# yerfor/Real3DPortrait

Hardware: AMD Instinct MI355X
Metric: rendered frames/sec @ 512x512, 48 depth samples (higher is better)
Workload: dtype f32 operands as fp16 hi + lo, fp32 accumulate (SR precision 'f16mx' = the library default, superresolution.DEFAULT_SR_PRECISION; the fp32-class f16x3 is `alt_f16x3`): in block0.conv1, block1.conv0 and block1.conv1 hi*hi runs on the f16 MFMA and the two cross products on the block-scaled 8-bit MFMA

## Files before the change

real3dportrait_amd/csrc/r3d_sr_f16x3.hip:

```cpp
#include <stdlib.h>

#include "r3d_sr_common.h"
#include "r3d_stamps.h"

namespace r3d {

typedef _Float16 h8 __attribute__((ext_vector_type(8)));
typedef _Float16 h4 __attribute__((ext_vector_type(4)));
static constexpr int F_TILE_H = 16, F_TILE_W = 16;
static constexpr int F_PATCH_H = F_TILE_H + 2, F_PATCH_W = F_TILE_W + 2, F_PATCH_PIX = F_PATCH_H * F_PATCH_W;

__device__ __forceinline__ void split1(float v, _Float16& hi, _Float16& lo)
{
    v = as_rounded(v);
    const float c = fminf(fmaxf(v, -65504.f), 65504.f);
    hi = (_Float16)c;
    lo = (_Float16)(v - (float)hi);
}

__device__ __forceinline__ void split1_folded(float v, _Float16& hi, _Float16& lo)
{
    v = as_rounded(v);
    hi = (_Float16)v;
    lo = (_Float16)(v - (float)hi);
}

__device__ __host__ __forceinline__ int mx_rec_chan(int dword) { return 8 * (dword & 1) + 4 * (dword >> 1); }
static constexpr float kMxWl = 256.0f , kMxWh = 0.125f ;
static constexpr int kMxFmtB = 1;
static constexpr int kMxScaleA = 127, kMxScaleB = 119;
static constexpr float kMxXh = 1.0f, kMxXl = 2048.0f ;

__device__ __forceinline__ unsigned pack4_fp8(float a, float b, float c, float d)
{
    int v = 0;
    v = __builtin_amdgcn_cvt_pk_fp8_f32(a, b, v, false);
    v = __builtin_amdgcn_cvt_pk_fp8_f32(c, d, v, true);
    return (unsigned)v;
}
__device__ __forceinline__ unsigned pack4_x8(float a, float b, float c, float d)
{
    int v = 0;
    v = __builtin_amdgcn_cvt_pk_bf8_f32(a, b, v, false);
    v = __builtin_amdgcn_cvt_pk_bf8_f32(c, d, v, true);
    return (unsigned)v;
}

__global__ void weight_row_stats_kernel(const float* __restrict__ w, int row_len, int CoutReal, int Cout, float* __restrict__ tail)
{
    const int co = blockIdx.x;
    const ConvTail T = conv_tail_layout(Cout);
    float mx = 0.f, l1 = 0.f;
    if (co < CoutReal)
// ... 794 lines not shown
    auto issue_w = [&](int st, u32x4& r) { r = *reinterpret_cast<const u32x4*>(WP + (size_t)(st < nst ? st : nst - 1) * 4 * a.Cout); };
    uint4* const Abuf = lds + 2 * BL_PATCH;
    const int aoff = h * 256 + 64 * wm + li;
    const int prow = li >> 4, row0 = wn * 2 * NT;
    int boff[NT];
#pragma unroll
    for (int nt = 0; nt < NT; ++nt) boff[nt] = h * 256 + (row0 + nt * 2 + prow) * 16 + (li & 15);

#pragma unroll
    for (int d = 0; d < BL_DEPTH; ++d) { issue(d, raw[d]); issue_w(d, wraw[d]); }
    stage_patch(0, raw[0], lds);
    *reinterpret_cast<u32x4*>(Abuf + threadIdx.x) = wraw[0];
    issue(BL_DEPTH, raw[0]); issue_w(BL_DEPTH, wraw[0]);
    asm volatile("s_waitcnt lgkmcnt(0)" ::: "memory");
    __builtin_amdgcn_s_barrier();
    asm volatile("" ::: "memory");
    for (int s0 = 0; s0 < nst; s0 += BL_DEPTH) {
#pragma unroll
        for (int d = 0; d < BL_DEPTH; ++d) {
            const int s = s0 + d;
            {
                const uint4* P = lds + (d & 1) * BL_PATCH;
                const uint4* A = Abuf + (d & 1) * 512 + aoff;
                h8 ah[2], al[2];
#pragma unroll
                for (int mt = 0; mt < 2; ++mt) { const uint4 q0 = A[32 * mt], q1 = A[128 + 32 * mt]; ah[mt] = *reinterpret_cast<const h8*>(&q0); al[mt] = *reinterpret_cast<const h8*>(&q1); }
                h8 bh[NT], bl[NT];
#pragma unroll
                for (int nt = 0; nt < NT; ++nt) { const uint4 r0 = P[boff[nt]], r1 = P[512 + boff[nt]]; bh[nt] = *reinterpret_cast<const h8*>(&r0); bl[nt] = *reinterpret_cast<const h8*>(&r1); }
#pragma unroll
                for (int nt = 0; nt < NT; ++nt)
#pragma unroll
                    for (int mt = 0; mt < 2; ++mt) {
                        acc[mt][nt] = __builtin_amdgcn_mfma_f32_32x32x16_f16(al[mt], bh[nt], acc[mt][nt], 0, 0, 0);
                        acc[mt][nt] = __builtin_amdgcn_mfma_f32_32x32x16_f16(ah[mt], bl[nt], acc[mt][nt], 0, 0, 0);
                        acc[mt][nt] = __builtin_amdgcn_mfma_f32_32x32x16_f16(ah[mt], bh[nt], acc[mt][nt], 0, 0, 0);
                    }
                stage_patch(s + 1, raw[(d + 1) % BL_DEPTH], lds + ((d + 1) & 1) * BL_PATCH);
                *reinterpret_cast<u32x4*>(Abuf + ((d + 1) & 1) * 512 + threadIdx.x) = wraw[(d + 1) % BL_DEPTH];
                issue(s + 1 + BL_DEPTH, raw[(d + 1) % BL_DEPTH]); issue_w(s + 1 + BL_DEPTH, wraw[(d + 1) % BL_DEPTH]);
                asm volatile("s_waitcnt lgkmcnt(0)" ::: "memory");
                __builtin_amdgcn_s_barrier();
                asm volatile("" ::: "memory");
            }
        }
    }
    conv_epilogue<WN, NT>(a, ph, n, acc, i0, j0, m0, reinterpret_cast<float*>(lds));
}

static constexpr int U_TILE = 14;
static constexpr int U_WSTAGE = 9 * 2 * 2 * 32;
static constexpr int U_PW = 17, U_PPLANE = 320;
static constexpr int U_PATCH = 4 * U_PPLANE;
static constexpr int U_STAGE = U_PATCH + U_WSTAGE;
static constexpr int U_LDS_UINT4 = 2 * U_STAGE + 2;
static constexpr int U_ZERO = 2 * U_STAGE;


struct UpArgs {
    const uint4* x; size_t x_stride_n;
    const uint4* wp;
    const float* out_scale; const float* bias; const float* next_scale; size_t vec_stride_n;
    uint4* y; size_t y_stride_n;
    int Cin, Cout, H, W, tiles_x, ntiles, tiles_per_xcd;
    float clamp;
    unsigned long long* clk;
};

__global__ void sr_prepack_up_kernel(const float* __restrict__ w, int Cin, int Cout, const float* __restrict__ winv, uint4* __restrict__ out)
{
    const size_t e = (size_t)blockIdx.x * blockDim.x + threadIdx.x;
    const size_t total = (size_t)9 * (Cin / 8) * Cout * 2;
    if (e >= total) return;
    const int co = e & 31, hl = (e >> 5) & 1, hc = (e >> 6) & 1;
    const int t = (int)((e >> 7) % 9);
    const size_t r = (e >> 7) / 9;
    const int nst = Cin / 16;
    const int st = (int)(r % nst), cg = (int)(r / nst);
    const int cout = cg * 32 + co;
    h8 v8;
#pragma unroll
    for (int j = 0; j < 8; ++j) {
        const int ci = st * 16 + hc * 8 + j;
        _Float16 a, b; split1(w[((size_t)cout * Cin + ci) * 9 + t] * (1.0f / winv[cout]), a, b);
        v8[j] = hl ? b : a;
    }
    out[e] = *reinterpret_cast<uint4*>(&v8);
}

__global__ void sr_prepack_up_mx_kernel(const float* __restrict__ w, int Cin, int Cout, const float* __restrict__ winv, uint4* __restrict__ out)
{
    const size_t e = (size_t)blockIdx.x * blockDim.x + threadIdx.x;
    const size_t total = (size_t)9 * (Cin / 8) * Cout * 2;
    if (e >= total) return;
    const int co = e & 31, hl = (e >> 5) & 1, hc = (e >> 6) & 1;
    const int t = (int)((e >> 7) % 9);
    const size_t r = (e >> 7) / 9;
    const int nst = Cin / 16;
    const int st = (int)(r % nst), cg = (int)(r / nst);
    const int cout = cg * 32 + co;
    const float ws = 1.0f / winv[cout];
    if (!hl) {
        h8 v8;
#pragma unroll
        for (int j = 0; j < 8; ++j) { _Float16 a, b; split1(w[((size_t)cout * Cin + st * 16 + hc * 8 + j) * 9 + t] * ws, a, b); v8[j] = a; }
        out[e] = *reinterpret_cast<uint4*>(&v8);
        return;
    }
    uint4 rec;
    unsigned* pr = reinterpret_cast<unsigned*>(&rec);
#pragma unroll
    for (int q = 0; q < 4; ++q) {
        float f[4];
#pragma unroll
        for (int j = 0; j < 4; ++j) {
            const float v = w[((size_t)cout * Cin + st * 16 + mx_rec_chan(q) + j) * 9 + t] * ws;
            _Float16 a, b; split1(v, a, b);
            f[j] = hc ? (float)a * kMxWh : (v - (float)a) * kMxWl;
        }
        pr[q] = pack4_fp8(f[0], f[1], f[2], f[3]);
    }
    out[e] = rec;
}

template <bool CLAMP, bool MX = false, bool MXIN = false, int NW = 4>
__global__ __launch_bounds__(64 * NW, NW == 8 ? 4 : 2) void upconv_fir_f16x3_kernel(UpArgs a)
{
    constexpr int NTL = 8 / NW;
    constexpr int NTHR = 64 * NW;
    R3D_STAMP_DECL;
    __shared__ uint4 lds[U_LDS_UINT4];
    const int G = a.Cout >> 5;
    const int xcd = blockIdx.x & 7, slot = blockIdx.x >> 3;
    const int tl = slot / G, cg = slot - tl * G;
    const int tile = xcd * a.tiles_per_xcd + tl;
    if (tile >= a.ntiles) return;
    const int n = blockIdx.y;
    if (blockIdx.x == (gridDim.x >> 1) && n == 0 && threadIdx.x == 0) clk_begin(kernarg_clk<UpArgs>());
    const int ty = tile / a.tiles_x, tx = tile - ty * a.tiles_x;
    const int i0 = ty * U_TILE, j0 = tx * U_TILE;
    const int tid = threadIdx.x, lane = tid & 63, wave = tid >> 6;
    const int li = lane & 31, h = lane >> 5;
    const int nst = a.Cin >> 4;
    const int chunk_stride = a.H * a.W;
    const size_t plane = (size_t)(a.Cin >> 3) * chunk_stride;
    const uint4* X = a.x + (size_t)n * a.x_stride_n;

    f32x16 acc[4][NTL];
#pragma unroll
    for (int p = 0; p < 4; ++p)
#pragma unroll
        for (int nt = 0; nt < NTL; ++nt)
#pragma unroll
            for (int r = 0; r < 16; ++r) acc[p][nt][r] = 0.f;

    const int prow = li >> 4, pcol = ((li & 15) - prow) & 15;
    const int row0 = wave * 2 * NTL;
    int boff[NTL];
#pragma unroll
    for (int nt = 0; nt < NTL; ++nt) boff[nt] = (row0 + nt * 2 + prow + 1) * U_PW + (pcol + 1) + h * U_PPLANE;
    const int aoff = U_PATCH + h * 64 + li;
    int b8c[NTL], b8r[NTL];
#pragma unroll
    for (int nt = 0; nt < NTL; ++nt) {
        const int pix = (row0 + nt * 2 + prow + 1) * U_PW + (pcol + 1) + 2 * U_PPLANE;
        b8c[nt] = pix - h; b8r[nt] = pix - h * U_PW;
    }
    const int a8d2 = U_PATCH + 32 + li + h * 256, a8d6 = U_PATCH + 32 + li + h * 768;
    const int a8c = U_PATCH + 32 + li + 4 * 128;
    if (MXIN && tid < 2) lds[U_ZERO + tid] = make_uint4(0, 0, 0, 0);

    const int wave_u = __builtin_amdgcn_readfirstlane(wave);
    constexpr int PK = (20 + NW - 1) / NW;
    constexpr int WKF = 18 / NW, WKR = 18 - WKF * NW;
    unsigned pf_off[PK];
    unsigned pf_valid = 0;
#pragma unroll
    for (int k = 0; k < PK; ++k) {
        const int sg = NW * k + wave_u, pc = sg / 5, idx = (sg - pc * 5) * 64 + lane;
        const int py = idx / U_PW, px = idx - py * U_PW;
        const int iy = i0 - 2 + py, ix = j0 - 2 + px;
        unsigned off = 0;
        if (sg < 20 && idx < U_PW * U_PW && iy >= 0 && iy < a.H && ix >= 0 && ix < a.W) {
            off = (unsigned)((pc >> 1) * plane) + (unsigned)((pc & 1) * chunk_stride + iy * a.W + ix);
            pf_valid |= 1u << k;
        }
        pf_off[k] = off;
    }
    const uint4* WP = a.wp + (size_t)cg * nst * U_WSTAGE;
    auto dma_stage = [&](int st, uint4* buf) {
        const uint4* src = WP + (size_t)st * U_WSTAGE + tid;
#pragma unroll
        for (int k = 0; k <= WKF; ++k)
            if (k < WKF || wave_u < WKR) dma64(src + NTHR * k, buf + U_PATCH + NTHR * k + 64 * wave_u);
        const uint4* Xs = X + (size_t)(2 * st) * chunk_stride;
#pragma unroll
        for (int k = 0; k < PK; ++k) {
            if (NW * k + wave_u < 20) {
                const uint4* g = (pf_valid & (1u << k)) ? Xs + pf_off[k] : g_zero16;
                dma64(g, buf + 64 * (NW * k + wave_u));
            }
        }
    };
    dma_stage(0, lds);
    R3D_STAMP(0);
    i8v pa68, pa17, pb68[NTL], pb17[NTL];
    for (int st = 0; st < nst; ++st) {
#ifdef R3D_STAMPS
        asm volatile("s_waitcnt lgkmcnt(0)" ::: "memory"); R3D_STAMP(1);
#endif
        asm volatile("s_waitcnt vmcnt(0) lgkmcnt(0)" ::: "memory");
        R3D_STAMP(4);
        __builtin_amdgcn_s_barrier();
        R3D_STAMP(5);
        asm volatile("" ::: "memory");
        const uint4* cur = lds + (st & 1) * U_STAGE;
        if (st + 1 < nst) dma_stage(st + 1, lds + ((st + 1) & 1) * U_STAGE);
        if constexpr (MXIN) {
            auto ld8 = [&](const uint4* p0, const uint4* p1) {
                const uint4 q0 = *p0, q1 = *p1;
                return (i8v){(int)q0.x, (int)q0.y, (int)q0.z, (int)q0.w, (int)q1.x, (int)q1.y, (int)q1.z, (int)q1.w};
            };
            auto ldh = [&](const uint4* p0) { uint4 q = *p0; return *reinterpret_cast<h8*>(&q); };
            const uint4* curA = cur + aoff;
            const int cb = (st & 1) * U_STAGE;
            h8 B1[2][NTL], A1[6];
#pragma unroll
            for (int nt = 0; nt < NTL; ++nt) { B1[0][nt] = ldh(cur + boff[nt]); B1[1][nt] = ldh(cur + boff[nt] - 1); }
            {
                constexpr int T1[6] = {0, 1, 3, 4, 2, 5};
#pragma unroll
                for (int k = 0; k < 6; ++k) A1[k] = ldh(curA + T1[k] * 128);
            }
            __builtin_amdgcn_sched_barrier(0);
            if (st > 0) {
#pragma unroll
                for (int nt = 0; nt < NTL; ++nt) {
                    acc[0][nt] = __builtin_amdgcn_mfma_scale_f32_32x32x64_f8f6f4(pa68, pb68[nt], acc[0][nt], 0, kMxFmtB, 0, kMxScaleA, 0, kMxScaleB);
                    acc[1][nt] = __builtin_amdgcn_mfma_scale_f32_32x32x64_f8f6f4(pa17, pb17[nt], acc[1][nt], 0, kMxFmtB, 0, kMxScaleA, 0, kMxScaleB);
                }
            }
            __builtin_amdgcn_sched_barrier(0);
            h8 B2[2][NTL], A2[3];
#pragma unroll
            for (int nt = 0; nt < NTL; ++nt) { B2[0][nt] = ldh(cur + boff[nt] - U_PW); B2[1][nt] = ldh(cur + boff[nt] - U_PW - 1); }
#pragma unroll
            for (int k = 0; k < 3; ++k) A2[k] = ldh(curA + (6 + k) * 128);
            __builtin_amdgcn_sched_barrier(0);
#pragma unroll
            for (int k = 0; k < 4; ++k)
#pragma unroll
                for (int nt = 0; nt < NTL; ++nt) acc[k][nt] = __builtin_amdgcn_mfma_f32_32x32x16_f16(A1[k], B1[0][nt], acc[k][nt], 0, 0, 0);
#pragma unroll
            for (int k = 0; k < 2; ++k)
#pragma unroll
                for (int nt = 0; nt < NTL; ++nt) acc[2 * k][nt] = __builtin_amdgcn_mfma_f32_32x32x16_f16(A1[4 + k], B1[1][nt], acc[2 * k][nt], 0, 0, 0);
            __builtin_amdgcn_sched_barrier(0);
            const i8v a02 = ld8(lds + cb + a8d2 + 0 * 128, lds + cb + a8d2 + 0 * 128 + 64);
            const i8v a35 = ld8(lds + cb + a8d2 + 3 * 128, lds + cb + a8d2 + 3 * 128 + 64);
            const i8v a4 = ld8(lds + (h ? U_ZERO : cb + a8c), lds + (h ? U_ZERO + 1 : cb + a8c + 64));
            i8v b3[NTL];
#pragma unroll
            for (int nt = 0; nt < NTL; ++nt) b3[nt] = ld8(cur + b8c[nt], cur + b8c[nt] + U_PPLANE);
            __builtin_amdgcn_sched_barrier(0);
#pragma unroll
            for (int k = 0; k < 2; ++k)
#pragma unroll
                for (int nt = 0; nt < NTL; ++nt) acc[k][nt] = __builtin_amdgcn_mfma_f32_32x32x16_f16(A2[k], B2[0][nt], acc[k][nt], 0, 0, 0);
#pragma unroll
            for (int nt = 0; nt < NTL; ++nt) acc[0][nt] = __builtin_amdgcn_mfma_f32_32x32x16_f16(A2[2], B2[1][nt], acc[0][nt], 0, 0, 0);
            __builtin_amdgcn_sched_barrier(0);
            pa68 = ld8(lds + cb + a8d2 + 6 * 128, lds + cb + a8d2 + 6 * 128 + 64);
            pa17 = ld8(lds + cb + a8d6 + 1 * 128, lds + cb + a8d6 + 1 * 128 + 64);
#pragma unroll
            for (int nt = 0; nt < NTL; ++nt) {
                pb68[nt] = ld8(cur + b8c[nt] - U_PW, cur + b8c[nt] - U_PW + U_PPLANE);
                pb17[nt] = ld8(cur + b8r[nt], cur + b8r[nt] + U_PPLANE);
            }
            __builtin_amdgcn_sched_barrier(0);
#pragma unroll
            for (int nt = 0; nt < NTL; ++nt) {
                acc[0][nt] = __builtin_amdgcn_mfma_scale_f32_32x32x64_f8f6f4(a02, b3[nt], acc[0][nt], 0, kMxFmtB, 0, kMxScaleA, 0, kMxScaleB);
                acc[2][nt] = __builtin_amdgcn_mfma_scale_f32_32x32x64_f8f6f4(a35, b3[nt], acc[2][nt], 0, kMxFmtB, 0, kMxScaleA, 0, kMxScaleB);
                acc[3][nt] = __builtin_amdgcn_mfma_scale_f32_32x32x64_f8f6f4(a4, b3[nt], acc[3][nt], 0, kMxFmtB, 0, kMxScaleA, 0, kMxScaleB);
            }
            __builtin_amdgcn_sched_barrier(0);
            continue;
        }
#pragma unroll
        for (int win = 0; win < 4; ++win) {
            const int sy = win >> 1, sx = win & 1;
            const int toff = -(sy * U_PW + sx);
            h8 bh[NTL], bl[NTL];
#pragma unroll
            for (int nt = 0; nt < NTL; ++nt) {
                uint4 r0 = cur[boff[nt] + toff];
                uint4 r1 = cur[boff[nt] + toff + 2 * U_PPLANE];
                bh[nt] = *reinterpret_cast<h8*>(&r0); bl[nt] = *reinterpret_cast<h8*>(&r1);
            }
#pragma unroll
            for (int ky = 2 * sy; ky <= (sy ? 2 : 1); ++ky)
#pragma unroll
                for (int kx = 2 * sx; kx <= (sx ? 2 : 1); ++kx) {
                    const int t = ky * 3 + kx, p = (ky & 1) * 2 + (kx & 1);
                    uint4 q0 = cur[t * 128 + aoff], q1 = cur[t * 128 + aoff + 32];
                    const h8 ah = *reinterpret_cast<h8*>(&q0), al = *reinterpret_cast<h8*>(&q1);
#pragma unroll
                    for (int nt = 0; nt < NTL; ++nt) {
                        acc[p][nt] = __builtin_amdgcn_mfma_f32_32x32x16_f16(al, bh[nt], acc[p][nt], 0, 0, 0);
                        acc[p][nt] = __builtin_amdgcn_mfma_f32_32x32x16_f16(ah, bl[nt], acc[p][nt], 0, 0, 0);
                        acc[p][nt] = __builtin_amdgcn_mfma_f32_32x32x16_f16(ah, bh[nt], acc[p][nt], 0, 0, 0);
                    }
                }
        }
    }
    if constexpr (MXIN) {
#pragma unroll
        for (int nt = 0; nt < NTL; ++nt) {
            acc[0][nt] = __builtin_amdgcn_mfma_scale_f32_32x32x64_f8f6f4(pa68, pb68[nt], acc[0][nt], 0, kMxFmtB, 0, kMxScaleA, 0, kMxScaleB);
            acc[1][nt] = __builtin_amdgcn_mfma_scale_f32_32x32x64_f8f6f4(pa17, pb17[nt], acc[1][nt], 0, kMxFmtB, 0, kMxScaleA, 0, kMxScaleB);
        }
    }

    R3D_STAMP(1);
    typedef float f2 __attribute__((ext_vector_type(2)));
    typedef _Float16 hh2 __attribute__((ext_vector_type(2)));
    float4* hls0 = reinterpret_cast<float4*>(lds);
    const int co0 = cg * 32;
    const float* D = a.out_scale + (size_t)n * a.vec_stride_n + co0;
    const float* Bv = a.bias + (size_t)n * a.vec_stride_n + co0;
    const float* NS = a.next_scale + (size_t)n * a.vec_stride_n + co0;
    const int OH = 2 * a.H, OW = 2 * a.W;
    const size_t oplane = (size_t)(a.Cout >> 3) * OH * OW;
    float4 dv4[4], bv4[4], nv4[4];
#pragma unroll
    for (int g = 0; g < 4; ++g) {
        dv4[g] = *reinterpret_cast<const float4*>(D + 8 * g + 4 * (tid & 1));
        bv4[g] = *reinterpret_cast<const float4*>(Bv + 8 * g + 4 * (tid & 1));
        nv4[g] = *reinterpret_cast<const float4*>(NS + 8 * g + 4 * (tid & 1));
    }
#pragma unroll
    for (int g = 0; g < 4; ++g)
        asm volatile("" :: "v"(dv4[g].x), "v"(dv4[g].w), "v"(bv4[g].x), "v"(bv4[g].w), "v"(nv4[g].x), "v"(nv4[g].w));
    __syncthreads();
    unsigned mxk_h[1024 / NTHR][2], mxk_l[1024 / NTHR][2];
#pragma unroll
    for (int k = 0; k < 1024 / NTHR; ++k) { mxk_h[k][0] = mxk_h[k][1] = 0u; mxk_l[k][0] = mxk_l[k][1] = 0u; }
#pragma unroll
    for (int g = 0; g < 4; ++g) {
        float4* hls = hls0 + (g & 1) * 2048;
#pragma unroll
        for (int pa = 0; pa < 2; ++pa)
#pragma unroll
            for (int nt = 0; nt < NTL; ++nt) {
                float hx[2][4];
#pragma unroll
                for (int r = 0; r < 4; ++r) {
                    const float t0 = acc[2 * pa][nt][4 * g + r], t1 = acc[2 * pa + 1][nt][4 * g + r];
                    const float ts = t0 + t1;
                    const float tsp1 = __builtin_bit_cast(float, __builtin_amdgcn_mov_dpp(__builtin_bit_cast(int, ts), 0x12F, 0xF, 0xF, true));
                    const float t0p1 = __builtin_bit_cast(float, __builtin_amdgcn_mov_dpp(__builtin_bit_cast(int, t0), 0x12F, 0xF, 0xF, true));
                    const float t1p1 = __builtin_bit_cast(float, __builtin_amdgcn_mov_dpp(__builtin_bit_cast(int, t1), 0x12F, 0xF, 0xF, true));
                    const float t0p2 = __builtin_bit_cast(float, __builtin_amdgcn_mov_dpp(__builtin_bit_cast(int, t0), 0x12E, 0xF, 0xF, true));
                    const float t1p2 = __builtin_bit_cast(float, __builtin_amdgcn_mov_dpp(__builtin_bit_cast(int, t1), 0x12E, 0xF, 0xF, true));
                    hx[0][r] = __builtin_fmaf(tsp1, 3.0f, t1 + t0p2);
                    hx[1][r] = __builtin_fmaf(t1p1 + t0p2, 3.0f, t0p1 + t1p2);
                }
                const int gy = row0 + nt * 2 + prow;
#pragma unroll
                for (int dx = 0; dx < 2; ++dx)
                    hls[((pa * 2 + h) * 16 + gy) * 32 + ((2 * pcol + dx + 8 * h) & 31)] = make_float4(hx[dx][0], hx[dx][1], hx[dx][2], hx[dx][3]);
            }
        __syncthreads();
        {
            const float4 b4 = bv4[g], n4 = nv4[g], d4 = dv4[g];
            const f2 ba = f2{b4.x, b4.y}, bb = f2{b4.z, b4.w};
            const f2 da = f2{d4.x, d4.y} * 0.0625f, db = f2{d4.z, d4.w} * 0.0625f;
            const float m = 1.4142135623730951f;
            const f2 ma = f2{n4.x, n4.y} * m, mb = f2{n4.z, n4.w} * m;
            uint4* d = a.y + (size_t)n * a.y_stride_n + (size_t)((co0 >> 3) + g) * OH * OW;
#pragma unroll
            for (int k = 0; k < 1024 / NTHR; ++k) {
                const int q = tid + NTHR * k;
                const int half = q & 1, oc = (q >> 1) & 31, rp = q >> 6;
                const bool live = rp < U_TILE && oc < 2 * U_TILE;
                f2 ha[5], hb[5];
#pragma unroll
                for (int rr = 0; rr < 5; ++rr) {
                    const int gyy = min(rp, U_TILE - 1) + ((rr + 1) >> 1);
                    const float4 t4 = hls[((((rr + 1) & 1) * 2 + half) * 16 + gyy) * 32 + ((oc + 8 * half) & 31)];
                    ha[rr] = f2{t4.x, t4.y}; hb[rr] = f2{t4.z, t4.w};
                }
#pragma unroll
                for (int dy = 0; dy < 2; ++dy) {
                    f2 va = ((ha[dy] + ha[dy + 3]) + (ha[dy + 1] + ha[dy + 2]) * 3.0f) * da + ba;
                    f2 vb = ((hb[dy] + hb[dy + 3]) + (hb[dy + 1] + hb[dy + 2]) * 3.0f) * db + bb;
                    va = __builtin_elementwise_max(va, va * 0.2f);
                    vb = __builtin_elementwise_max(vb, vb * 0.2f);
                    if constexpr (CLAMP) {
                        const f2 lim = f2{a.clamp, a.clamp} * 0.7071067811865476f;
                        va = __builtin_elementwise_min(__builtin_elementwise_max(va, -lim), lim);
                        vb = __builtin_elementwise_min(__builtin_elementwise_max(vb, -lim), lim);
                    }
                    va = va * ma;
                    vb = vb * mb;
                    asm("" : "+v"(va), "+v"(vb));
                    const hh2 hia = __builtin_convertvector(va, hh2), hib = __builtin_convertvector(vb, hh2);
                    const hh2 loa = __builtin_convertvector(va - __builtin_convertvector(hia, f2), hh2);
                    const hh2 lob = __builtin_convertvector(vb - __builtin_convertvector(hib, f2), hh2);
                    const uint2 hw = make_uint2(*reinterpret_cast<const unsigned*>(&hia), *reinterpret_cast<const unsigned*>(&hib));
                    const int oy = 2 * (i0 + rp) + dy, ox = 2 * j0 + oc;
                    if constexpr (MX) {
                        const f2 fha = __builtin_convertvector(hia, f2), fhb = __builtin_convertvector(hib, f2);
                        const f2 fla = va - fha, flb = vb - fhb;
                        const unsigned xh8 = pack4_x8(fha.x * kMxXh, fha.y * kMxXh, fhb.x * kMxXh, fhb.y * kMxXh);
                        const unsigned xl8 = pack4_x8(fla.x * kMxXl, fla.y * kMxXl, flb.x * kMxXl, flb.y * kMxXl);
                        if (!(g & 1)) { mxk_h[k][dy] = xh8; mxk_l[k][dy] = xl8; }
                        if (live && oy < OH && ox < OW) {
                            const size_t pix = (size_t)oy * OW + ox;
                            reinterpret_cast<uint2*>(d + pix)[half] = hw;
                            if (g & 1) {
                                uint4* rec = a.y + (size_t)n * a.y_stride_n + oplane + (size_t)((co0 >> 3) + (g & ~1)) * OH * OW + pix;
                                reinterpret_cast<uint2*>(rec)[half] = make_uint2(mxk_h[k][dy], xh8);
                                reinterpret_cast<uint2*>(rec + (size_t)OH * OW)[half] = make_uint2(mxk_l[k][dy], xl8);
                            }
                        }
                    } else {
                        const uint2 lw = make_uint2(*reinterpret_cast<const unsigned*>(&loa), *reinterpret_cast<const unsigned*>(&lob));
                        if (live && oy < OH && ox < OW) {
                            uint2* d2 = reinterpret_cast<uint2*>(d + (size_t)oy * OW + ox) + half;
                            d2[0] = hw;
                            d2[2 * oplane] = lw;
                        }
                    }
                }
            }
        }
    }
    R3D_STAMP(2);
    if (blockIdx.x == (gridDim.x >> 1) && blockIdx.y == 0 && threadIdx.x == 0) clk_end(kernarg_clk<UpArgs>());
#ifdef R3D_STAMPS
    asm volatile("s_waitcnt vmcnt(0)" ::: "memory");
    R3D_STAMP(3);
    R3D_STAMP_FLUSH(6, 1);
#endif
}
R3D_STAMP_READER(r3d_debug_stamps_sr)

__global__ void rgb_finalize_kernel(const float* __restrict__ img_prev, const float* __restrict__ partial, size_t part_stride_n,
                                    int nparts, const float* __restrict__ brgb, size_t vec_stride_n,
                                    float* __restrict__ img_out, uint8_t* __restrict__ img_u8, int H, int W, float clamp, int up)
{
    const int n = blockIdx.y;
    const int p = blockIdx.x * blockDim.x + threadIdx.x;
    if (p >= H * W) return;
    const int y = p / W, xx = p - y * W;
    const int Hh = H >> 1, Wh = W >> 1;
    const int ky = y >> 1, kx = xx >> 1;
    int r0, r1, c0, c1; float wy0, wy1, wx0, wx1;
    if (y & 1) { r0 = ky; r1 = ky + 1; wy0 = 0.75f; wy1 = 0.25f; } else { r0 = ky - 1; r1 = ky; wy0 = 0.25f; wy1 = 0.75f; }
    if (xx & 1) { c0 = kx; c1 = kx + 1; wx0 = 0.75f; wx1 = 0.25f; } else { c0 = kx - 1; c1 = kx; wx0 = 0.25f; wx1 = 0.75f; }
    const bool vr0 = r0 >= 0 && r0 < Hh, vr1 = r1 >= 0 && r1 < Hh, vc0 = c0 >= 0 && c0 < Wh, vc1 = c1 >= 0 && c1 < Wh;
    float rgb[3];
#pragma unroll
    for (int c = 0; c < 3; ++c) {
        float t = brgb[(size_t)n * vec_stride_n + c];
        for (int m = 0; m < nparts; ++m) t += partial[(size_t)n * part_stride_n + ((size_t)m * 3 + c) * H * W + p];
        if (clamp >= 0.f) t = fminf(fmaxf(t, -clamp), clamp);
        float upv;
        if (up) {
            const float* I = img_prev + ((size_t)n * 3 + c) * Hh * Wh;
            upv = 0.f;
            if (vr0 && vc0) upv += I[(size_t)r0 * Wh + c0] * (wy0 * wx0);
            if (vr0 && vc1) upv += I[(size_t)r0 * Wh + c1] * (wy0 * wx1);
            if (vr1 && vc0) upv += I[(size_t)r1 * Wh + c0] * (wy1 * wx0);
            if (vr1 && vc1) upv += I[(size_t)r1 * Wh + c1] * (wy1 * wx1);
        } else {
            upv = img_prev[((size_t)n * 3 + c) * H * W + p];
        }
        rgb[c] = upv + t;
        if (img_out) img_out[((size_t)n * 3 + c) * H * W + p] = rgb[c];
    }
    if (img_u8) {
        uint8_t* d = img_u8 + ((size_t)n * H * W + p) * 3;
#pragma unroll
        for (int c = 0; c < 3; ++c) d[c] = frame_u8(rgb[c]);
    }
}

__global__ void cb8_to_nchw2_kernel(const float* __restrict__ src, float* __restrict__ dst, int C, int HW)
{
    const int n = blockIdx.z, cb = blockIdx.y;
    const int p = blockIdx.x * blockDim.x + threadIdx.x;
// ... 153 lines not shown
    const size_t mu = (size_t)9 * (Cin / 8) * Cout * 2;
    hipLaunchKernelGGL(sr_prepack_up_kernel, dim3((unsigned)((mu + 255) / 256)), dim3(256), 0, st, c0_w, Cin, Cout, tail0 + T.winv,
                       reinterpret_cast<uint4*>(out + P.c0_up));
    if (mx) {
        hipLaunchKernelGGL(sr_prepack_up_mx_kernel, dim3((unsigned)((mu + 255) / 256)), dim3(256), 0, st, c0_w, Cin, Cout, tail0 + T.winv,
                           reinterpret_cast<uint4*>(out + P.c0_up_mx));
        if ((Cin & 15) == 0)
            hipLaunchKernelGGL(sr_prepack_mx_kernel, dim3((unsigned)((m0 / 2 + 255) / 256)), dim3(256), 0, st, c0_w, Cin, Cout, 9, Cin, Cout,
                               tail0 + T.winv, reinterpret_cast<uint4*>(out + P.c0_mx));
    }
    {
        const size_t mw = (size_t)(Cout >> 7) * (Cout >> 4) * 8 * 3 * 2 * 32;
        hipLaunchKernelGGL(sr_prepack_wino_kernel, dim3((unsigned)((mw + 255) / 256)), dim3(256), 0, st, c1_w, Cout, Cout, Cout, Cout, tail1 + T.winv,
                           reinterpret_cast<uint4*>(out + P.c1_wino), mx ? 1 : 0);
    }
    return check_launch("sr_block_prepack");
}

static void launch_conv2(Conv2Args& a, int tiles, int N, hipStream_t st, bool mx = false, bool wino = false)
{
    a.clk = prof_clock_slot(R3D_PROF_CONV);
    dim3 grid(tiles, a.Cout / BLOCK_M, N);
    a.order = (tiles & 7) == 0 ? 2 : 0;
    if (wino) {
        if (mx) hipLaunchKernelGGL(conv_wino_f16x3_kernel<true>, grid, dim3(512), 0, st, a);
        else hipLaunchKernelGGL(conv_wino_f16x3_kernel<false>, grid, dim3(512), 0, st, a);
        return;
    }
    if (a.ph[0].ntaps == 9 && (size_t)tiles * grid.y * grid.z <= 256) {
        const int t8 = ((a.ph[0].outW + F_TILE_W - 1) / F_TILE_W) * ((a.ph[0].outH + 7) / 8);
        a.order = (t8 & 7) == 0 ? 2 : 0;
        if (mx) hipLaunchKernelGGL(conv_mfma_f16x3_rows8_kernel<true>, dim3(t8, grid.y, grid.z), dim3(512), 0, st, a);
        else hipLaunchKernelGGL(conv_mfma_f16x3_rows8_kernel<false>, dim3(t8, grid.y, grid.z), dim3(512), 0, st, a);
        return;
    }
    if (a.ph[0].ntaps == 1) hipLaunchKernelGGL((conv1x1_mfma_f16x3_kernel<4, 2, 4>), grid, dim3(512), 0, st, a);
    else if (mx) hipLaunchKernelGGL((conv_mfma_f16x3_kernel<4, 2, 4, true>), grid, dim3(512), 0, st, a);
    else hipLaunchKernelGGL((conv_mfma_f16x3_kernel<4, 2, 4>), grid, dim3(512), 0, st, a);
}

static int tiles_of(int H, int W) { return ((W + F_TILE_W - 1) / F_TILE_W) * ((H + F_TILE_H - 1) / F_TILE_H); }

static void conv_set_output(Conv2Args& a, void* y, int y_format, int Cout, int H, int W, const float* next_scale, size_t next_scale_stride)
{
    if (y_format == R3D_FMT_CB8) { a.y_f32 = reinterpret_cast<float*>(y); a.y_f32_stride_n = (size_t)Cout * H * W; }
    else if (y_format == R3D_FMT_NCHW) { a.y_nchw = reinterpret_cast<float*>(y); a.y_nchw_stride_n = (size_t)Cout * H * W; }
    else if (y_format == R3D_FMT_SPLIT || y_format == R3D_FMT_SPLIT_MX) {
        a.y_split = reinterpret_cast<uint4*>(y); a.y_split_stride_n = (size_t)Cout / 8 * H * W * 2;
        a.next_scale = next_scale; a.next_scale_stride_n = next_scale_stride;
        a.y_split_mx = y_format == R3D_FMT_SPLIT_MX ? 1 : 0;
    }
}

static void (*const kUpconv[2][2][2])(UpArgs) = {
    {{upconv_fir_f16x3_kernel<false, false, false>, upconv_fir_f16x3_kernel<false, false, true>}, {upconv_fir_f16x3_kernel<false, true, false>, upconv_fir_f16x3_kernel<false, true, true>}},
    {{upconv_fir_f16x3_kernel<true, false, false>, upconv_fir_f16x3_kernel<true, false, true>}, {upconv_fir_f16x3_kernel<true, true, false>, upconv_fir_f16x3_kernel<true, true, true>}}};

int sr_block_forward_f16x3(const void* prepacked, const void* styles, int N, int Cin, int Cout, int Hin, int Win, int up,
                           const void* x, int x_format, const float* img, float clamp,
                           void* x_out, int x_out_format, const float* next_scale, size_t next_scale_stride,
                           float* img_out, uint8_t* img_u8, float* x_absmax, void* workspace, hipStream_t st, bool mx)
{
    const SrStyleLayout L = sr_style_layout(Cin, Cout);
    const float* pk = reinterpret_cast<const float*>(styles);
    const float* wpk = reinterpret_cast<const float*>(prepacked);
    const SrPackLayout P = sr_pack_layout(Cin, Cout);
    const int OH = up ? 2 * Hin : Hin, OW = up ? 2 * Win : Win;
    const SrWorkspaceLayout WS = sr_workspace_layout(N, Cin, Cout, Hin, Win);
    char* wsb = reinterpret_cast<char*>(workspace);
    uint4* xin = reinterpret_cast<uint4*>(wsb + WS.xin);
    uint4* y0 = reinterpret_cast<uint4*>(wsb + WS.y0);
    float* rgbp = reinterpret_cast<float*>(wsb + WS.rgbp);

    const uint4* xs = reinterpret_cast<const uint4*>(x);
    const bool mx_in = x_format == R3D_FMT_SPLIT_MX;
    if (x_format != R3D_FMT_SPLIT && !mx_in) {
        ProfScope ps(R3D_PROF_LAYOUT, st);
        hipLaunchKernelGGL(to_split_kernel, dim3((Hin * Win + 255) / 256, Cin / 8, N), dim3(256), 0, st,
                           reinterpret_cast<const float*>(x), x_format == R3D_FMT_CB8 ? 1 : 0, pk + L.s0f, L.total, xin, Cin, Cin, Hin * Win);
        xs = xin;
    }
    const bool wino1 = wino_shape_ok(Cout, Cout, OH, OW) && (wino_mode() == 1 || (wino_mode() == 2 && mx) || (wino_mode() == 3 && !mx));
    const bool mx0 = mx && !wino1;
    if (up) {
        UpArgs u = {};
        u.x = xs; u.x_stride_n = (size_t)Cin / 8 * Hin * Win * 2;
        u.wp = reinterpret_cast<const uint4*>(wpk + (mx_in ? P.c0_up_mx : P.c0_up));
        u.out_scale = pk + L.d0f; u.bias = pk + L.b0; u.next_scale = pk + L.s1f; u.vec_stride_n = L.total;
        u.y = y0; u.y_stride_n = (size_t)Cout / 8 * OH * OW * 2;
        u.Cin = Cin; u.Cout = Cout; u.H = Hin; u.W = Win;
        u.tiles_x = (Win + U_TILE - 1) / U_TILE;
        u.ntiles = u.tiles_x * ((Hin + U_TILE - 1) / U_TILE);
        u.tiles_per_xcd = (u.ntiles + 7) / 8;
        u.clamp = clamp;
        u.clk = prof_clock_slot(R3D_PROF_UPCONV);
        ProfScope ps(R3D_PROF_UPCONV, st);
        const dim3 ugrid(8 * u.tiles_per_xcd * (Cout / 32), N);
        hipLaunchKernelGGL(kUpconv[clamp >= 0.f][mx0][mx_in], ugrid, dim3(256), 0, st, u);
    } else {
        Conv2Args a = {};
        a.x = xs; a.x_stride_n = (size_t)Cin / 8 * Hin * Win * 2;
        a.wp = reinterpret_cast<const uint4*>(wpk + (mx_in ? P.c0_mx : P.c0));
        a.out_scale = pk + L.d0f; a.out_scale_stride_n = L.total; a.bias = pk + L.b0; a.bias_stride_n = L.total;
        a.OH = OH; a.OW = OW;
        conv_set_output(a, y0, mx0 ? R3D_FMT_SPLIT_MX : R3D_FMT_SPLIT, Cout, OH, OW, pk + L.s1f, L.total);
        a.Cin = Cin; a.Cout = Cout; a.CoutReal = Cout; a.H = Hin; a.W = Win; a.nphase = 1;
        a.act = 1; a.act_slope = 0.2f; a.act_gain = 1.4142135623730951f; a.clamp = clamp;
        sr_fill_conv3x3_phase(a.ph, OH, OW);
        ProfScope ps(R3D_PROF_CONV, st);
        launch_conv2(a, tiles_of(OH, OW), N, st, mx_in);
    }
    {
        Conv2Args a = {};
        a.x = y0; a.x_stride_n = (size_t)Cout / 8 * OH * OW * 2;
        a.wp = reinterpret_cast<const uint4*>(wpk + (wino1 ? P.c1_wino : P.c1));
        a.out_scale = pk + L.d1f; a.out_scale_stride_n = L.total; a.bias = pk + L.b1; a.bias_stride_n = L.total;
        a.OH = OH; a.OW = OW;
        if (x_out) conv_set_output(a, x_out, x_out_format, Cout, OH, OW, next_scale, next_scale_stride);
        a.y_absmax = reinterpret_cast<unsigned*>(x_absmax);
        a.wrgb = pk + L.wrgb; a.wrgb_stride_n = L.total; a.rgb_partial = rgbp; a.rgbp_stride_n = (size_t)(Cout / 64) * 3 * OH * OW;
        a.Cin = Cout; a.Cout = Cout; a.CoutReal = Cout; a.H = OH; a.W = OW; a.nphase = 1;
        a.act = 1; a.act_slope = 0.2f; a.act_gain = 1.4142135623730951f; a.clamp = clamp;
        sr_fill_conv3x3_phase(a.ph, OH, OW);
        ProfScope ps(R3D_PROF_CONV, st);
        launch_conv2(a, tiles_of(OH, OW), N, st, mx, wino1);
    }
    {
        ProfScope ps(R3D_PROF_TORGB, st);
        hipLaunchKernelGGL(rgb_finalize_kernel, dim3((OH * OW + 255) / 256, N), dim3(256), 0, st, img, rgbp,
                           (size_t)(Cout / 64) * 3 * OH * OW, Cout / 64, pk + L.brgb, L.total, img_out, img_u8, OH, OW, clamp, up);
    }
    return check_launch("sr_block_forward(f16x3)");
}

size_t conv_prepacked_bytes_f16x3(int Cin, int Cout, int ksize) { return conv_pack_layout(Cin, Cout, ksize).total * sizeof(float); }

int conv_prepack_f16x3(const float* w, int Cin, int Cout, int ksize, void* prepacked, hipStream_t st)
{
    const ConvPackLayout P = conv_pack_layout(Cin, Cout, ksize);
    const int Ci = P.Ci, Co = P.Co, nt = ksize * ksize;
    const size_t m = (size_t)nt * (Ci / 8) * Co;
    float* out = reinterpret_cast<float*>(prepacked);
    float* tail = out + P.tail;
    ProfScope ps(R3D_PROF_PACK, st);
    hipLaunchKernelGGL(weight_row_stats_kernel, dim3(Co), dim3(256), 0, st, w, Cin * nt, Cout, Co, tail);
    hipLaunchKernelGGL(sr_prepack_f16_kernel, dim3((unsigned)((m + 255) / 256)), dim3(256), 0, st, w, Cin, Cout, nt, Ci, Co,
                       tail + conv_tail_layout(Co).winv, reinterpret_cast<uint4*>(out + P.w));
    if (ksize == 3) {
        hipLaunchKernelGGL(sr_prepack_mx_kernel, dim3((unsigned)((m / 2 + 255) / 256)), dim3(256), 0, st, w, Cin, Cout, nt, Ci, Co,
                           tail + conv_tail_layout(Co).winv, reinterpret_cast<uint4*>(out + P.w_mx));
        const size_t mw = (size_t)(Co >> 7) * (Ci >> 4) * 8 * 3 * 2 * 32;
// ... 73 lines not shown
```

Before: 1750.

## Make upconv kernel persistent with 8 waves covering 64 output channels

The upsampling conv kernel becomes persistent. The grid is capped at the CU count, and each block loops over (batch, tile, channel-group) work items, prefetching the next item's first stage into the spare LDS buffer during the last K-stage of the current one. Each block now uses 8 waves split into two 32-channel halves. This lets the patch load be shared across 64 output channels, and the epilogue vectors are staged through LDS. The aim is to remove launch tail and prologue bubbles and to halve activation reloads per channel. In exchange the kernel uses more LDS and registers and the epilogue control is more complex.

```diff
diff --git a/real3dportrait_amd/csrc/r3d_sr_f16x3.hip b/real3dportrait_amd/csrc/r3d_sr_f16x3.hip
--- a/real3dportrait_amd/csrc/r3d_sr_f16x3.hip
+++ b/real3dportrait_amd/csrc/r3d_sr_f16x3.hip
@@ -1,4 +1,7 @@
 #include <stdlib.h>
+
+#include <algorithm>
+#include <atomic>
 
 #include "r3d_sr_common.h"
 #include "r3d_stamps.h"
@@ -899,9 +902,12 @@
 static constexpr int U_WSTAGE = 9 * 2 * 2 * 32;
 static constexpr int U_PW = 17, U_PPLANE = 320;
 static constexpr int U_PATCH = 4 * U_PPLANE;
-static constexpr int U_STAGE = U_PATCH + U_WSTAGE;
-static constexpr int U_LDS_UINT4 = 2 * U_STAGE + 2;
-static constexpr int U_ZERO = 2 * U_STAGE;
+static constexpr int U_STAGE = U_PATCH + 2 * U_WSTAGE;
+static constexpr int U_HSLICE = 2048;
+static constexpr int U_H1 = 2 * U_STAGE;
+static constexpr int U_VEC = U_H1 + U_HSLICE;
+static constexpr int U_ZERO = U_VEC + 48;
+static constexpr int U_LDS_UINT4 = U_ZERO + 2;
 
 
 struct UpArgs {
@@ -909,7 +915,7 @@
     const uint4* wp;
     const float* out_scale; const float* bias; const float* next_scale; size_t vec_stride_n;
     uint4* y; size_t y_stride_n;
-    int Cin, Cout, H, W, tiles_x, ntiles, tiles_per_xcd;
+    int Cin, Cout, H, W, tiles_x, ntiles, tiles_per_xcd, N;
     float clamp;
     unsigned long long* clk;
 };
@@ -970,76 +976,74 @@
     out[e] = rec;
 }
 
-template <bool CLAMP, bool MX = false, bool MXIN = false, int NW = 4>
-__global__ __launch_bounds__(64 * NW, NW == 8 ? 4 : 2) void upconv_fir_f16x3_kernel(UpArgs a)
-{
-    constexpr int NTL = 8 / NW;
+template <bool CLAMP, bool MX = false, bool MXIN = false, int NW = 8>
+__global__ __launch_bounds__(64 * NW, 2) void upconv_fir_f16x3_kernel(UpArgs a)
+{
+    static_assert(NW == 8, "two cout halves x four row groups");
+    constexpr int NTL = 2;
     constexpr int NTHR = 64 * NW;
     R3D_STAMP_DECL;
     __shared__ uint4 lds[U_LDS_UINT4];
-    const int G = a.Cout >> 5;
-    const int xcd = blockIdx.x & 7, slot = blockIdx.x >> 3;
-    const int tl = slot / G, cg = slot - tl * G;
-    const int tile = xcd * a.tiles_per_xcd + tl;
-    if (tile >= a.ntiles) return;
-    const int n = blockIdx.y;
-    if (blockIdx.x == (gridDim.x >> 1) && n == 0 && threadIdx.x == 0) clk_begin(kernarg_clk<UpArgs>());
-    const int ty = tile / a.tiles_x, tx = tile - ty * a.tiles_x;
-    const int i0 = ty * U_TILE, j0 = tx * U_TILE;
-    const int tid = threadIdx.x, lane = tid & 63, wave = tid >> 6;
-    const int li = lane & 31, h = lane >> 5;
+    const int G = a.Cout >> 6;
+    const int per_n = 8 * a.tiles_per_xcd * G, total = per_n * a.N;
+    const int wave_u = __builtin_amdgcn_readfirstlane((int)threadIdx.x >> 6);
+    const int wm = wave_u >> 2, wq = wave_u & 3;
+    auto opaque_tid = [] { int t = threadIdx.x; asm volatile("" : "+v"(t)); return t; };
+    typedef const __attribute__((address_space(4))) UpArgs* KA;
+    auto kernargs = [] { KA ap = (KA)__builtin_amdgcn_kernarg_segment_ptr(); asm volatile("" : "+s"(ap)); return ap; };
     const int nst = a.Cin >> 4;
     const int chunk_stride = a.H * a.W;
     const size_t plane = (size_t)(a.Cin >> 3) * chunk_stride;
-    const uint4* X = a.x + (size_t)n * a.x_stride_n;
-
-    f32x16 acc[4][NTL];
-#pragma unroll
-    for (int p = 0; p < 4; ++p)
-#pragma unroll
-        for (int nt = 0; nt < NTL; ++nt)
-#pragma unroll
-            for (int r = 0; r < 16; ++r) acc[p][nt][r] = 0.f;
-
-    const int prow = li >> 4, pcol = ((li & 15) - prow) & 15;
-    const int row0 = wave * 2 * NTL;
-    int boff[NTL];
-#pragma unroll
-    for (int nt = 0; nt < NTL; ++nt) boff[nt] = (row0 + nt * 2 + prow + 1) * U_PW + (pcol + 1) + h * U_PPLANE;
-    const int aoff = U_PATCH + h * 64 + li;
-    int b8c[NTL], b8r[NTL];
-#pragma unroll
-    for (int nt = 0; nt < NTL; ++nt) {
-        const int pix = (row0 + nt * 2 + prow + 1) * U_PW + (pcol + 1) + 2 * U_PPLANE;
-        b8c[nt] = pix - h; b8r[nt] = pix - h * U_PW;
-    }
-    const int a8d2 = U_PATCH + 32 + li + h * 256, a8d6 = U_PATCH + 32 + li + h * 768;
-    const int a8c = U_PATCH + 32 + li + 4 * 128;
-    if (MXIN && tid < 2) lds[U_ZERO + tid] = make_uint4(0, 0, 0, 0);
-
-    const int wave_u = __builtin_amdgcn_readfirstlane(wave);
-    constexpr int PK = (20 + NW - 1) / NW;
-    constexpr int WKF = 18 / NW, WKR = 18 - WKF * NW;
+    auto decode = [&](int it, int& n_, int& tile_, int& cg_) {
+        n_ = it / per_n;
+        const int rem = it - n_ * per_n, xcd = rem & 7, slot = rem >> 3, tl = slot / G;
+        cg_ = slot - tl * G; tile_ = xcd * a.tiles_per_xcd + tl;
+    };
+    auto next_item = [&](int it) {
+        for (; it < total; it += (int)gridDim.x) { int n_, tile_, cg_; decode(it, n_, tile_, cg_); if (tile_ < a.ntiles) break; }
+        return it;
+    };
+    int it = next_item(blockIdx.x);
+    if (it >= total) return;
+    const bool sampler = blockIdx.x == (gridDim.x >> 1) && threadIdx.x == 0;
+    if (sampler) clk_begin(kernarg_clk<UpArgs>());
+
+    if (MXIN && threadIdx.x < 2) lds[U_ZERO + threadIdx.x] = make_uint4(0, 0, 0, 0);
+
+    constexpr int PK = 3;
     unsigned pf_off[PK];
     unsigned pf_valid = 0;
-#pragma unroll
-    for (int k = 0; k < PK; ++k) {
-        const int sg = NW * k + wave_u, pc = sg / 5, idx = (sg - pc * 5) * 64 + lane;
-        const int py = idx / U_PW, px = idx - py * U_PW;
-        const int iy = i0 - 2 + py, ix = j0 - 2 + px;
-        unsigned off = 0;
-        if (sg < 20 && idx < U_PW * U_PW && iy >= 0 && iy < a.H && ix >= 0 && ix < a.W) {
-            off = (unsigned)((pc >> 1) * plane) + (unsigned)((pc & 1) * chunk_stride + iy * a.W + ix);
-            pf_valid |= 1u << k;
-        }
-        pf_off[k] = off;
-    }
-    const uint4* WP = a.wp + (size_t)cg * nst * U_WSTAGE;
+    const uint4* X; const uint4* WP;
+    auto dma_setup = [&](int n_, int tile_, int cg_) {
+        const int ty = tile_ / a.tiles_x, tx = tile_ - ty * a.tiles_x;
+        const int lane = opaque_tid() & 63;
+        const KA ka = kernargs();
+        pf_valid = 0;
+#pragma unroll
+        for (int k = 0; k < PK; ++k) {
+            const int sg = NW * k + wave_u, pc = sg / 5, idx = (sg - pc * 5) * 64 + lane;
+            const int py = idx / U_PW, px = idx - py * U_PW;
+            const int iy = ty * U_TILE - 2 + py, ix = tx * U_TILE - 2 + px;
+            unsigned off = 0;
+            if (sg < 20 && idx < U_PW * U_PW && iy >= 0 && iy < a.H && ix >= 0 && ix < a.W) {
+                off = (unsigned)((pc >> 1) * plane) + (unsigned)((pc & 1) * chunk_stride + iy * a.W + ix);
+                pf_valid |= 1u << k;
+            }
+            pf_off[k] = off;
+        }
+        X = ka->x + (size_t)n_ * ka->x_stride_n;
+        WP = ka->wp + (size_t)(2 * cg_) * nst * U_WSTAGE;
+    };
     auto dma_stage = [&](int st, uint4* buf) {
-        const uint4* src = WP + (size_t)st * U_WSTAGE + tid;
-#pragma unroll
-        for (int k = 0; k <= WKF; ++k)
-            if (k < WKF || wave_u < WKR) dma64(src + NTHR * k, buf + U_PATCH + NTHR * k + 64 * wave_u);
+        const uint4* src = WP + (size_t)st * U_WSTAGE + (opaque_tid() & 63);
+#pragma unroll
+        for (int k = 0; k < 5; ++k) {
+            const int s = NW * k + wave_u;
+            if (s < 36) {
+                const int grp = s >= 18 ? 1 : 0;
+                dma64(src + (size_t)grp * nst * U_WSTAGE + (s - 18 * grp) * 64, buf + U_PATCH + 64 * s);
+            }
+        }
         const uint4* Xs = X + (size_t)(2 * st) * chunk_stride;
 #pragma unroll
         for (int k = 0; k < PK; ++k) {
@@ -1049,9 +1053,41 @@
             }
         }
     };
+    int n, tile, cg;
+    decode(it, n, tile, cg);
+    dma_setup(n, tile, cg);
+    int par = 0;
     dma_stage(0, lds);
+    bool first = true;
+  for (;;) {
     R3D_STAMP(0);
+    dma_setup(n, tile, cg);
+    const int tid = opaque_tid(), li = tid & 31, h = (tid >> 5) & 1;
+    const int prow = li >> 4, pcol = ((li & 15) - prow) & 15;
+    const int row0 = wq * 2 * NTL;
+    int boff[NTL];
+#pragma unroll
+    for (int nt = 0; nt < NTL; ++nt) boff[nt] = (row0 + nt * 2 + prow + 1) * U_PW + (pcol + 1) + h * U_PPLANE;
+    const int aoff = U_PATCH + wm * U_WSTAGE + h * 64 + li;
+    int b8c[NTL], b8r[NTL];
+#pragma unroll
+    for (int nt = 0; nt < NTL; ++nt) {
+        const int pix = (row0 + nt * 2 + prow + 1) * U_PW + (pcol + 1) + 2 * U_PPLANE;
+        b8c[nt] = pix - h; b8r[nt] = pix - h * U_PW;
+    }
+    const int a8d2 = U_PATCH + wm * U_WSTAGE + 32 + li + h * 256, a8d6 = U_PATCH + wm * U_WSTAGE + 32 + li + h * 768;
+    const int a8c = U_PATCH + wm * U_WSTAGE + 32 + li + 4 * 128;
+    const int i0 = (tile / a.tiles_x) * U_TILE, j0 = (tile - (tile / a.tiles_x) * a.tiles_x) * U_TILE;
+    int nx = total, nn = 0, ntile = 0, ncg = 0;
+    f32x16 acc[4][NTL];
+#pragma unroll
+    for (int p = 0; p < 4; ++p)
+#pragma unroll
+        for (int nt = 0; nt < NTL; ++nt)
+#pragma unroll
+            for (int r = 0; r < 16; ++r) acc[p][nt][r] = 0.f;
     i8v pa68, pa17, pb68[NTL], pb17[NTL];
+    float4 vec_ld = make_float4(0.f, 0.f, 0.f, 0.f);
     for (int st = 0; st < nst; ++st) {
 #ifdef R3D_STAMPS
         asm volatile("s_waitcnt lgkmcnt(0)" ::: "memory"); R3D_STAMP(1);
@@ -1061,8 +1097,20 @@
         __builtin_amdgcn_s_barrier();
         R3D_STAMP(5);
         asm volatile("" ::: "memory");
-        const uint4* cur = lds + (st & 1) * U_STAGE;
-        if (st + 1 < nst) dma_stage(st + 1, lds + ((st + 1) & 1) * U_STAGE);
+        const int cb = ((par + st) & 1) * U_STAGE;
+        const uint4* cur = lds + cb;
+        uint4* oth = lds + (U_STAGE - cb);
+        if (st + 1 < nst) dma_stage(st + 1, oth);
+        else {
+            nx = next_item(it + (int)gridDim.x);
+            if (nx < total) { decode(nx, nn, ntile, ncg); dma_setup(nn, ntile, ncg); dma_stage(0, oth); }
+            const int tv = opaque_tid();
+            if (tv < 48) {
+                const KA ka = kernargs();
+                const float* V = tv < 16 ? ka->out_scale : tv < 32 ? ka->bias : ka->next_scale;
+                vec_ld = *reinterpret_cast<const float4*>(V + (size_t)n * ka->vec_stride_n + cg * 64 + (tv & 15) * 4);
+            }
+        }
         if constexpr (MXIN) {
             auto ld8 = [&](const uint4* p0, const uint4* p1) {
                 const uint4 q0 = *p0, q1 = *p1;
@@ -1070,7 +1118,6 @@
             };
             auto ldh = [&](const uint4* p0) { uint4 q = *p0; return *reinterpret_cast<h8*>(&q); };
             const uint4* curA = cur + aoff;
-            const int cb = (st & 1) * U_STAGE;
             h8 B1[2][NTL], A1[6];
 #pragma unroll
             for (int nt = 0; nt < NTL; ++nt) { B1[0][nt] = ldh(cur + boff[nt]); B1[1][nt] = ldh(cur + boff[nt] - 1); }
@@ -1167,35 +1214,29 @@
             acc[0][nt] = __builtin_amdgcn_mfma_scale_f32_32x32x64_f8f6f4(pa68, pb68[nt], acc[0][nt], 0, kMxFmtB, 0, kMxScaleA, 0, kMxScaleB);
             acc[1][nt] = __builtin_amdgcn_mfma_scale_f32_32x32x64_f8f6f4(pa17, pb17[nt], acc[1][nt], 0, kMxFmtB, 0, kMxScaleA, 0, kMxScaleB);
         }
+#pragma unroll
+        for (int nt = 0; nt < NTL; ++nt) asm volatile("" : "+v"(acc[0][nt]), "+v"(acc[1][nt]), "+v"(acc[2][nt]), "+v"(acc[3][nt]));
     }
 
     R3D_STAMP(1);
+  {
+    const int tid = opaque_tid(), li = tid & 31, h = (tid >> 5) & 1, prow = li >> 4, pcol = ((li & 15) - prow) & 15;
+    const KA ka = kernargs();
     typedef float f2 __attribute__((ext_vector_type(2)));
     typedef _Float16 hh2 __attribute__((ext_vector_type(2)));
-    float4* hls0 = reinterpret_cast<float4*>(lds);
-    const int co0 = cg * 32;
-    const float* D = a.out_scale + (size_t)n * a.vec_stride_n + co0;
-    const float* Bv = a.bias + (size_t)n * a.vec_stride_n + co0;
-    const float* NS = a.next_scale + (size_t)n * a.vec_stride_n + co0;
+    float4* const hbuf0 = reinterpret_cast<float4*>(lds + ((par + nst - 1) & 1) * U_STAGE);
+    float4* const hbuf1 = reinterpret_cast<float4*>(lds + U_H1);
+    const int co0 = cg * 64;
     const int OH = 2 * a.H, OW = 2 * a.W;
     const size_t oplane = (size_t)(a.Cout >> 3) * OH * OW;
-    float4 dv4[4], bv4[4], nv4[4];
+    if (tid < 48) reinterpret_cast<float4*>(lds + U_VEC)[tid] = vec_ld;
+    asm volatile("s_waitcnt lgkmcnt(0)" ::: "memory");
+    __builtin_amdgcn_s_barrier();
+    asm volatile("" ::: "memory");
+    unsigned mxk_h[2][1024 / NTHR][2], mxk_l[2][1024 / NTHR][2];
 #pragma unroll
     for (int g = 0; g < 4; ++g) {
-        dv4[g] = *reinterpret_cast<const float4*>(D + 8 * g + 4 * (tid & 1));
-        bv4[g] = *reinterpret_cast<const float4*>(Bv + 8 * g + 4 * (tid & 1));
-        nv4[g] = *reinterpret_cast<const float4*>(NS + 8 * g + 4 * (tid & 1));
-    }
-#pragma unroll
-    for (int g = 0; g < 4; ++g)
-        asm volatile("" :: "v"(dv4[g].x), "v"(dv4[g].w), "v"(bv4[g].x), "v"(bv4[g].w), "v"(nv4[g].x), "v"(nv4[g].w));
-    __syncthreads();
-    unsigned mxk_h[1024 / NTHR][2], mxk_l[1024 / NTHR][2];
-#pragma unroll
-    for (int k = 0; k < 1024 / NTHR; ++k) { mxk_h[k][0] = mxk_h[k][1] = 0u; mxk_l[k][0] = mxk_l[k][1] = 0u; }
-#pragma unroll
-    for (int g = 0; g < 4; ++g) {
-        float4* hls = hls0 + (g & 1) * 2048;
+        float4* hls = wm ? hbuf1 : hbuf0;
 #pragma unroll
         for (int pa = 0; pa < 2; ++pa)
 #pragma unroll
@@ -1218,14 +1259,19 @@
                 for (int dx = 0; dx < 2; ++dx)
                     hls[((pa * 2 + h) * 16 + gy) * 32 + ((2 * pcol + dx + 8 * h) & 31)] = make_float4(hx[dx][0], hx[dx][1], hx[dx][2], hx[dx][3]);
             }
-        __syncthreads();
-        {
-            const float4 b4 = bv4[g], n4 = nv4[g], d4 = dv4[g];
+        asm volatile("s_waitcnt lgkmcnt(0)" ::: "memory");
+        __builtin_amdgcn_s_barrier();
+        asm volatile("" ::: "memory");
+#pragma unroll
+        for (int hs = 0; hs < 2; ++hs) {
+            hls = hs ? hbuf1 : hbuf0;
+            const float4* vec = reinterpret_cast<const float4*>(lds + U_VEC) + hs * 8 + 2 * g + (tid & 1);
+            const float4 d4 = vec[0], b4 = vec[16], n4 = vec[32];
             const f2 ba = f2{b4.x, b4.y}, bb = f2{b4.z, b4.w};
             const f2 da = f2{d4.x, d4.y} * 0.0625f, db = f2{d4.z, d4.w} * 0.0625f;
             const float m = 1.4142135623730951f;
             const f2 ma = f2{n4.x, n4.y} * m, mb = f2{n4.z, n4.w} * m;
-            uint4* d = a.y + (size_t)n * a.y_stride_n + (size_t)((co0 >> 3) + g) * OH * OW;
+            char* const d = reinterpret_cast<char*>(ka->y + (size_t)n * ka->y_stride_n + (size_t)((co0 >> 3) + 4 * hs + g) * OH * OW);
 #pragma unroll
             for (int k = 0; k < 1024 / NTHR; ++k) {
                 const int q = tid + NTHR * k;
@@ -1262,30 +1308,40 @@
                         const f2 fla = va - fha, flb = vb - fhb;
                         const unsigned xh8 = pack4_x8(fha.x * kMxXh, fha.y * kMxXh, fhb.x * kMxXh, fhb.y * kMxXh);
                         const unsigned xl8 = pack4_x8(fla.x * kMxXl, fla.y * kMxXl, flb.x * kMxXl, flb.y * kMxXl);
-                        if (!(g & 1)) { mxk_h[k][dy] = xh8; mxk_l[k][dy] = xl8; }
+                        if (!(g & 1)) { mxk_h[hs][k][dy] = xh8; mxk_l[hs][k][dy] = xl8; }
                         if (live && oy < OH && ox < OW) {
-                            const size_t pix = (size_t)oy * OW + ox;
-                            reinterpret_cast<uint2*>(d + pix)[half] = hw;
+                            const unsigned voff = (unsigned)(oy * OW + ox) * 16u + 8u * half;
+                            *reinterpret_cast<uint2*>(d + voff) = hw;
                             if (g & 1) {
-                                uint4* rec = a.y + (size_t)n * a.y_stride_n + oplane + (size_t)((co0 >> 3) + (g & ~1)) * OH * OW + pix;
-                                reinterpret_cast<uint2*>(rec)[half] = make_uint2(mxk_h[k][dy], xh8);
-                                reinterpret_cast<uint2*>(rec + (size_t)OH * OW)[half] = make_uint2(mxk_l[k][dy], xl8);
+                                char* const rec = reinterpret_cast<char*>(ka->y + (size_t)n * ka->y_stride_n + oplane + (size_t)((co0 >> 3) + 4 * hs + (g & ~1)) * OH * OW);
+                                *reinterpret_cast<uint2*>(rec + voff) = make_uint2(mxk_h[hs][k][dy], xh8);
+                                *reinterpret_cast<uint2*>(rec + (size_t)OH * OW * 16 + voff) = make_uint2(mxk_l[hs][k][dy], xl8);
                             }
                         }
                     } else {
                         const uint2 lw = make_uint2(*reinterpret_cast<const unsigned*>(&loa), *reinterpret_cast<const unsigned*>(&lob));
                         if (live && oy < OH && ox < OW) {
-                            uint2* d2 = reinterpret_cast<uint2*>(d + (size_t)oy * OW + ox) + half;
-                            d2[0] = hw;
-                            d2[2 * oplane] = lw;
+                            const unsigned voff = (unsigned)(oy * OW + ox) * 16u + 8u * half;
+                            *reinterpret_cast<uint2*>(d + voff) = hw;
+                            *reinterpret_cast<uint2*>(d + oplane * 16 + voff) = lw;
                         }
                     }
                 }
             }
         }
-    }
+        if (g < 3) {
+            asm volatile("s_waitcnt lgkmcnt(0)" ::: "memory");
+            __builtin_amdgcn_s_barrier();
+            asm volatile("" ::: "memory");
+        }
+    }
+  }
     R3D_STAMP(2);
-    if (blockIdx.x == (gridDim.x >> 1) && blockIdx.y == 0 && threadIdx.x == 0) clk_end(kernarg_clk<UpArgs>());
+    if (first && sampler) clk_end(kernarg_clk<UpArgs>());
+    first = false;
+    if (nx >= total) break;
+    it = nx; n = nn; tile = ntile; cg = ncg; par = (par + nst) & 1;
+  }
 #ifdef R3D_STAMPS
     asm volatile("s_waitcnt vmcnt(0)" ::: "memory");
     R3D_STAMP(3);
@@ -1545,6 +1601,19 @@
     }
 }
 
+static int upconv_cu_count()
+{
+    static std::atomic<int> cus[64];
+    int dev = 0;
+    if (hipGetDevice(&dev) != hipSuccess || dev < 0 || dev >= 64) dev = 0;
+    int v = cus[dev].load(std::memory_order_relaxed);
+    if (v <= 0) {
+        if (hipDeviceGetAttribute(&v, hipDeviceAttributeMultiprocessorCount, dev) != hipSuccess || v <= 0) v = 8;
+        cus[dev].store(v, std::memory_order_relaxed);
+    }
+    return v;
+}
+
 static void (*const kUpconv[2][2][2])(UpArgs) = {
     {{upconv_fir_f16x3_kernel<false, false, false>, upconv_fir_f16x3_kernel<false, false, true>}, {upconv_fir_f16x3_kernel<false, true, false>, upconv_fir_f16x3_kernel<false, true, true>}},
     {{upconv_fir_f16x3_kernel<true, false, false>, upconv_fir_f16x3_kernel<true, false, true>}, {upconv_fir_f16x3_kernel<true, true, false>, upconv_fir_f16x3_kernel<true, true, true>}}};
@@ -1588,8 +1657,10 @@
         u.clamp = clamp;
         u.clk = prof_clock_slot(R3D_PROF_UPCONV);
         ProfScope ps(R3D_PROF_UPCONV, st);
-        const dim3 ugrid(8 * u.tiles_per_xcd * (Cout / 32), N);
-        hipLaunchKernelGGL(kUpconv[clamp >= 0.f][mx0][mx_in], ugrid, dim3(256), 0, st, u);
+        u.N = N;
+        const int items = 8 * u.tiles_per_xcd * (Cout / 64) * N;
+        const int ugrid = std::min(items, std::max(8, upconv_cu_count() & ~7));
+        hipLaunchKernelGGL(kUpconv[clamp >= 0.f][mx0][mx_in], dim3(ugrid), dim3(512), 0, st, u);
     } else {
         Conv2Args a = {};
         a.x = xs; a.x_stride_n = (size_t)Cin / 8 * Hin * Win * 2;
```

New measurement: 1708. -2.4%, worse.
